# chinhau5/parallel_eda

Hardware: AMD Instinct MI355X
Metric: place+route wall-clock to feasibility (s/flow; bitcoin_miner-scale synthetic on stratixiv-like fabric) (lower is better)
Workload: dtype fp32; 1 GPU; model=bitcoin_miner, arch=bitcoin_stratixiv, grid=280x200, W=300, rr_nodes=15745036, rr_edges=87277236, blocks=37632, nets=35616, conns=110426, global_batch=110426, seq_len=0, final_overused=0, wirelength=4913966

## Files before the change

csrc/hip/place_kernel.hip:

```cpp
#include "pnr_hip.h"

namespace pnrh {

struct PlaceDev {
  const int32_t* net_blk_ptr;
  const int32_t* net_blks;
  const int32_t* blk_net_ptr;
  const int32_t* blk_nets;
  const int8_t* blk_type;
  const int8_t* tile_btype;
  const int32_t* type_cols;
  const int32_t* type_col_ptr;
  const uint8_t* fixed;
  const float* net_q;
  const int32_t* net_sink_ptr;
  const float* conn_crit;
  const float* delay_mat;
  int32_t* bx;
  int32_t* by;
  int32_t* bslot;
  int32_t* grid;
  float* net_cost;
  float* net_tcost;
  int32_t num_blocks, num_nets, gx, gy, cap, nx, ny, io_cap;
// ... 170 lines not shown
                     ? (p.tile_btype[tx * p.gy + ty] != p.blk_type[b])
                     : (is_io_loc(p, tx, ty) != (p.blk_type[b] == 0))) ok = 0;
        else if (cap_at(p, tx, ty) != 1) ok = 0;
        else {
          int32_t occ = p.grid[((int64_t)tx * p.gy + ty) * p.cap];
          if (occ >= 0 && p.macro_of[occ] != mid) ok = 0;
        }
      }
      if (ok) atomicAdd(&m.counters[0], 1);
    }
    ok = __shfl(ok, 0);
    if (!ok) return;
    float dbb = 0.0f, dtd = 0.0f;
    for (int32_t j = mm0; j < mm1; ++j) {
      int32_t b = p.macro_blk[j];
      for (int32_t k = p.blk_net_ptr[b] + lane; k < p.blk_net_ptr[b + 1];
           k += 64) {
        int32_t n = p.blk_nets[k];
        bool dup = false;
        for (int32_t j2 = mm0; j2 < j && !dup; ++j2)
          dup = blk_has_net(p, p.macro_blk[j2], n);
        if (dup) continue;
        dbb += net_bb_cost_macro(p, n, mid, ddx, ddy) - p.net_cost[n];
        if (timing_tradeoff > 0.0f)
          dtd += net_td_cost_macro(p, n, mid, ddx, ddy) - p.net_tcost[n];
      }
    }
    dbb = wave_sum_f32(dbb);
    dtd = wave_sum_f32(dtd);
    float delta = (1.0f - timing_tradeoff) * dbb * inv_bb_norm +
                  timing_tradeoff * dtd * inv_td_norm;
    bool accept;
    if (delta <= 0.0f) accept = true;
    else if (T <= 0.0f) accept = false;
    else {
      float u = (rng_hash(seed, batch, i * 131 + 5) & 0xFFFFFF) *
                (1.0f / 16777216.0f);
      accept = u < __expf(-delta / T);
    }
    if (!accept) return;
    if (lane == 0) {
      atomicAdd(&m.counters[1], 1);
      m.mv_blk[i] = blk;
      m.mv_to[i] = ((ddx + 4096) << 13) | (ddy + 4096);
      m.mv_other[i] = -2 - mid;
      m.mv_dbb[i] = dbb;
      m.mv_dtd[i] = dtd;
      m.mv_flags[i] = 1;
    }
    for (int32_t j = mm0; j < mm1; ++j) {
      int32_t b = p.macro_blk[j];
      for (int32_t k = p.blk_net_ptr[b] + lane; k < p.blk_net_ptr[b + 1];
           k += 64)
        atomicMin(&m.net_claim[p.blk_nets[k]], i);
    }
    for (int32_t j = mm0 + lane; j < mm1; j += 64) {
      int32_t b = p.macro_blk[j];
      atomicMin(&m.loc_claim[p.bx[b] * p.gy + p.by[b]], i);
      atomicMin(&m.loc_claim[(p.bx[b] + ddx) * p.gy + p.by[b] + ddy], i);
    }
    return;
  }
  int32_t other = p.grid[((int64_t)x1 * p.gy + y1) * p.cap + slot1];
  if (other == blk) return;
  if (other >= 0 && p.fixed && p.fixed[other]) return;
  if (other >= 0 && p.macro_of && p.macro_of[other] >= 0)
    return;
  if (lane == 0) atomicAdd(&m.counters[0], 1);
  float dbb = 0.0f, dtd = 0.0f;
  const int ox = other >= 0 ? x0 : -1000, oy = other >= 0 ? y0 : -1000;
  for (int32_t k = p.blk_net_ptr[blk] + lane; k < p.blk_net_ptr[blk + 1];
       k += 64) {
    int32_t n = p.blk_nets[k];
    dbb += net_bb_cost(p, n, blk, x1, y1, other, ox, oy) - p.net_cost[n];
    if (timing_tradeoff > 0.0f)
      dtd += net_td_cost(p, n, blk, x1, y1, other, ox, oy) - p.net_tcost[n];
  }
  if (other >= 0) {
    for (int32_t k = p.blk_net_ptr[other] + lane;
         k < p.blk_net_ptr[other + 1]; k += 64) {
      int32_t n = p.blk_nets[k];
      if (blk_has_net(p, blk, n)) continue;
      dbb += net_bb_cost(p, n, blk, x1, y1, other, ox, oy) - p.net_cost[n];
      if (timing_tradeoff > 0.0f)
        dtd += net_td_cost(p, n, blk, x1, y1, other, ox, oy) - p.net_tcost[n];
    }
  }
  dbb = wave_sum_f32(dbb);
  dtd = wave_sum_f32(dtd);
  float delta = (1.0f - timing_tradeoff) * dbb * inv_bb_norm +
                timing_tradeoff * dtd * inv_td_norm;
  bool accept;
  if (delta <= 0.0f) accept = true;
  else if (T <= 0.0f) accept = false;
  else {
    float u = (rng_hash(seed, batch, i * 131 + 5) & 0xFFFFFF) *
              (1.0f / 16777216.0f);
    accept = u < __expf(-delta / T);
  }
  if (!accept) return;
  if (lane == 0) {
    atomicAdd(&m.counters[1], 1);
    m.mv_blk[i] = blk;
    m.mv_to[i] = ((x1 * p.gy + y1) * p.cap + slot1);
    m.mv_other[i] = other;
    m.mv_dbb[i] = dbb;
    m.mv_dtd[i] = dtd;
    m.mv_flags[i] = 1;
    atomicMin(&m.loc_claim[x0 * p.gy + y0], i);
    atomicMin(&m.loc_claim[x1 * p.gy + y1], i);
  }
  for (int32_t k = p.blk_net_ptr[blk] + lane; k < p.blk_net_ptr[blk + 1];
       k += 64)
    atomicMin(&m.net_claim[p.blk_nets[k]], i);
  if (other >= 0)
    for (int32_t k = p.blk_net_ptr[other] + lane;
         k < p.blk_net_ptr[other + 1]; k += 64)
      atomicMin(&m.net_claim[p.blk_nets[k]], i);
}

__device__ int propose_select_impl(const PlaceDev& p, int rlim,
                                   uint32_t seed, uint32_t batch, int i,
                                   int& x1o, int& y1o, int& slot1o) {
  uint32_t r0 = rng_hash(seed ^ 0x5BD1E995u, batch, i);
  int32_t blk = r0 % p.num_blocks;
  if (p.fixed && p.fixed[blk]) return -1;
  if (p.rx0 >= 0 && (p.bx[blk] < p.rx0 || p.bx[blk] > p.rx1))
    return -1;
  bool io = p.blk_type[blk] == 0;
  int x0 = p.bx[blk], y0 = p.by[blk];
  int x1 = -1, y1 = -1, slot1 = 0;
  int bt = p.blk_type[blk];
  if (p.tile_btype && bt >= 2 && p.type_cols) {
    int c0 = p.type_col_ptr[bt - 2], c1 = p.type_col_ptr[bt - 1];
    int lo = c0, hi = c1;
    while (lo < hi) { int m = (lo + hi) >> 1;
                      if (p.type_cols[m] < x0 - rlim) lo = m + 1; else hi = m; }
    int lo2 = lo, hi2 = c1;
    while (lo2 < hi2) { int m = (lo2 + hi2) >> 1;
                        if (p.type_cols[m] <= x0 + rlim) lo2 = m + 1; else hi2 = m; }
    int ncol = lo2 - lo;
    if (ncol > 0) {
      int ylo = max(1, y0 - rlim), yhi = min(p.ny, y0 + rlim);
      for (int att = 0; att < 8; ++att) {
        uint32_t r1 = rng_hash(seed, batch, i * 131 + 7 * att + 1);
        uint32_t r2 = rng_hash(seed, batch, i * 131 + 7 * att + 2);
        int tx = p.type_cols[lo + (int)(r1 % ncol)];
        if (p.rx0 >= 0 && (tx < p.rx0 || tx > p.rx1)) continue;
        int ty = ylo + (int)(r2 % (yhi - ylo + 1));
        if (tx == x0 && ty == y0) continue;
        x1 = tx; y1 = ty; slot1 = 0;
        break;
      }
    }
  } else {
    for (int att = 0; att < 8; ++att) {
      uint32_t r1 = rng_hash(seed, batch, i * 131 + 7 * att + 1);
      uint32_t r2 = rng_hash(seed, batch, i * 131 + 7 * att + 2);
      int tx = x0 + (int)(r1 % (2 * rlim + 1)) - rlim;
      int ty = y0 + (int)(r2 % (2 * rlim + 1)) - rlim;
      if (tx < 0 || tx >= p.gx || ty < 0 || ty >= p.gy) continue;
      if (p.rx0 >= 0 && (tx < p.rx0 || tx > p.rx1)) continue;
      if (p.tile_btype) {
        if (p.tile_btype[tx * p.gy + ty] != p.blk_type[blk]) continue;
      } else if (is_io_loc(p, tx, ty) != io) continue;
      int c = cap_at(p, tx, ty);
      if (c <= 0) continue;
      if (tx == x0 && ty == y0) continue;
      x1 = tx; y1 = ty;
      slot1 = (int)(rng_hash(seed, batch, i * 131 + 7 * att + 3) % c);
      break;
    }
  }
  if (x1 < 0) return -1;
  x1o = x1; y1o = y1; slot1o = slot1;
  return blk;
}

__launch_bounds__(64 * PROP_WAVES, 2)
__global__ void place_resolve_kernel(PlaceDev p, MovesDev m) {
  const int lane = threadIdx.x & 63;
  const int i = blockIdx.x * PROP_WAVES + (threadIdx.x >> 6);
  if (i >= m.n_moves || m.mv_flags[i] != 1) return;
  int32_t blk = m.mv_blk[i];
  int32_t other = m.mv_other[i];
  int32_t to = m.mv_to[i];
  bool bad = false;
  if (other <= -2) {
    const int mid = -2 - other;
    const int ddx = (to >> 13) - 4096, ddy = (to & 0x1FFF) - 4096;
    const int32_t mm0 = p.macro_ptr[mid], mm1 = p.macro_ptr[mid + 1];
    for (int32_t j = mm0 + lane; j < mm1; j += 64) {
      int32_t b = p.macro_blk[j];
      int sx = p.bx[b], sy = p.by[b];
      if (m.loc_claim[sx * p.gy + sy] != i ||
          m.loc_claim[(sx + ddx) * p.gy + sy + ddy] != i) bad = true;
    }
    for (int32_t j = mm0; j < mm1; ++j) {
      int32_t b = p.macro_blk[j];
      for (int32_t k = p.blk_net_ptr[b] + lane; k < p.blk_net_ptr[b + 1];
           k += 64)
        if (m.net_claim[p.blk_nets[k]] != i) bad = true;
    }
  } else {
    int x1 = to / p.cap / p.gy, y1 = (to / p.cap) % p.gy;
    int x0 = p.bx[blk], y0 = p.by[blk];
    if (lane == 0 && (m.loc_claim[x0 * p.gy + y0] != i ||
                      m.loc_claim[x1 * p.gy + y1] != i)) bad = true;
    for (int32_t k = p.blk_net_ptr[blk] + lane; k < p.blk_net_ptr[blk + 1];
         k += 64)
      if (m.net_claim[p.blk_nets[k]] != i) bad = true;
    if (other >= 0)
      for (int32_t k = p.blk_net_ptr[other] + lane;
           k < p.blk_net_ptr[other + 1]; k += 64)
        if (m.net_claim[p.blk_nets[k]] != i) bad = true;
  }
  const bool win = !__any(bad);
  if (lane == 0) {
    if (!win) { m.mv_flags[i] = 0; atomicAdd(&m.counters[3], 1); }
    else { m.mv_flags[i] = 2; atomicAdd(&m.counters[2], 1); }
  }
}

__launch_bounds__(64 * PROP_WAVES, 2)
__global__ void place_apply_kernel(PlaceDev p, MovesDev m, float timing_tradeoff,
                                   double* cost_acc ) {
  const int lane = threadIdx.x & 63;
  const int i = blockIdx.x * PROP_WAVES + (threadIdx.x >> 6);
  if (i >= m.n_moves || m.mv_flags[i] != 2) return;
  int32_t blk = m.mv_blk[i];
  int32_t other = m.mv_other[i];
  int32_t to = m.mv_to[i];
  if (other <= -2) {
    const int mid = -2 - other;
    const int ddx = (to >> 13) - 4096, ddy = (to & 0x1FFF) - 4096;
    const int32_t mm0 = p.macro_ptr[mid], mm1 = p.macro_ptr[mid + 1];
    for (int32_t j = mm0; j < mm1; ++j) {
      int32_t b = p.macro_blk[j];
      for (int32_t k = p.blk_net_ptr[b] + lane; k < p.blk_net_ptr[b + 1];
           k += 64) {
        int32_t n = p.blk_nets[k];
        p.net_cost[n] = net_bb_cost_macro(p, n, mid, ddx, ddy);
        if (timing_tradeoff > 0.0f)
          p.net_tcost[n] = net_td_cost_macro(p, n, mid, ddx, ddy);
      }
    }
    if (lane == 0) {
      for (int32_t j = mm0; j < mm1; ++j) {
        int32_t b = p.macro_blk[j];
        p.grid[((int64_t)p.bx[b] * p.gy + p.by[b]) * p.cap + p.bslot[b]] = -1;
      }
      for (int32_t j = mm0; j < mm1; ++j) {
        int32_t b = p.macro_blk[j];
        int tx = p.bx[b] + ddx, ty = p.by[b] + ddy;
        p.grid[((int64_t)tx * p.gy + ty) * p.cap] = b;
        p.bx[b] = tx; p.by[b] = ty; p.bslot[b] = 0;
      }
      unsafeAtomicAdd(&cost_acc[0], (double)m.mv_dbb[i]);
      unsafeAtomicAdd(&cost_acc[1], (double)m.mv_dtd[i]);
    }
    return;
  }
  int slot1 = to % p.cap;
  int x1 = to / p.cap / p.gy, y1 = (to / p.cap) % p.gy;
  int x0 = p.bx[blk], y0 = p.by[blk], s0 = p.bslot[blk];
  const int ox = other >= 0 ? x0 : -1000, oy = other >= 0 ? y0 : -1000;
  for (int32_t k = p.blk_net_ptr[blk] + lane; k < p.blk_net_ptr[blk + 1];
       k += 64) {
    int32_t n = p.blk_nets[k];
    p.net_cost[n] = net_bb_cost(p, n, blk, x1, y1, other, ox, oy);
    if (timing_tradeoff > 0.0f)
      p.net_tcost[n] = net_td_cost(p, n, blk, x1, y1, other, ox, oy);
  }
  if (other >= 0)
    for (int32_t k = p.blk_net_ptr[other] + lane;
         k < p.blk_net_ptr[other + 1]; k += 64) {
      int32_t n = p.blk_nets[k];
      p.net_cost[n] = net_bb_cost(p, n, blk, x1, y1, other, ox, oy);
      if (timing_tradeoff > 0.0f)
        p.net_tcost[n] = net_td_cost(p, n, blk, x1, y1, other, ox, oy);
    }
  if (lane == 0) {
    p.grid[((int64_t)x0 * p.gy + y0) * p.cap + s0] = other >= 0 ? other : -1;
    p.grid[((int64_t)x1 * p.gy + y1) * p.cap + slot1] = blk;
    p.bx[blk] = x1; p.by[blk] = y1; p.bslot[blk] = slot1;
    if (other >= 0) { p.bx[other] = x0; p.by[other] = y0; p.bslot[other] = s0; }
    unsafeAtomicAdd(&cost_acc[0], (double)m.mv_dbb[i]);
    unsafeAtomicAdd(&cost_acc[1], (double)m.mv_dtd[i]);
  }
}

__global__ void place_reset_claims_kernel(int32_t* net_claim, int32_t nn,
                                          int32_t* loc_claim, int32_t nl,
                                          int32_t* counters) {
  int i = blockIdx.x * blockDim.x + threadIdx.x;
  int total = max(nn, nl);
  (void)counters;
  for (; i < total; i += gridDim.x * blockDim.x) {
    if (i < nn) net_claim[i] = 0x7FFFFFFF;
    if (i < nl) loc_claim[i] = 0x7FFFFFFF;
  }
}

__global__ void place_refresh_costs_kernel(PlaceDev p, float timing_tradeoff,
                                           double* out ) {
  int n = blockIdx.x * blockDim.x + threadIdx.x;
  for (; n < p.num_nets; n += gridDim.x * blockDim.x) {
    float c = net_bb_cost(p, n, -1, 0, 0, -1, 0, 0);
    p.net_cost[n] = c;
    unsafeAtomicAdd(&out[0], (double)c);
    float t = (timing_tradeoff > 0.0f)
                  ? net_td_cost(p, n, -1, 0, 0, -1, 0, 0) : 0.0f;
    p.net_tcost[n] = t;
    unsafeAtomicAdd(&out[1], (double)t);
  }
}

}

using namespace pnrh;

extern "C" {

struct PlaceLaunchArgs {
  const int32_t* net_blk_ptr; const int32_t* net_blks;
  const int32_t* blk_net_ptr; const int32_t* blk_nets;
  const int8_t* blk_type; const int8_t* tile_btype;
  const int32_t* type_cols; const int32_t* type_col_ptr;
  const uint8_t* fixed;
  const float* net_q;
  const int32_t* net_sink_ptr; const float* conn_crit; const float* delay_mat;
  int32_t* bx; int32_t* by; int32_t* bslot; int32_t* grid;
  float* net_cost; float* net_tcost;
  int32_t num_blocks, num_nets, gx, gy, cap, nx, ny, io_cap;
  int32_t rx0, rx1;
  const int32_t* macro_of; const int32_t* macro_ptr;
  const int32_t* macro_blk;
  int32_t* mv_blk; int32_t* mv_to; int32_t* mv_other;
  float* mv_dbb; float* mv_dtd; uint8_t* mv_flags;
  int32_t* net_claim; int32_t* loc_claim; int32_t* counters;
  int32_t n_moves;
  float T; int32_t rlim; float timing_tradeoff;
  float inv_bb_norm, inv_td_norm;
  uint32_t seed, batch;
  double* cost_acc;
};

static void unpack(const PlaceLaunchArgs* a, PlaceDev& p, MovesDev& m) {
  p.net_blk_ptr = a->net_blk_ptr; p.net_blks = a->net_blks;
  p.blk_net_ptr = a->blk_net_ptr; p.blk_nets = a->blk_nets;
  p.blk_type = a->blk_type; p.tile_btype = a->tile_btype;
  p.type_cols = a->type_cols; p.type_col_ptr = a->type_col_ptr;
  p.fixed = a->fixed;
  p.net_q = a->net_q;
  p.net_sink_ptr = a->net_sink_ptr; p.conn_crit = a->conn_crit;
  p.delay_mat = a->delay_mat;
  p.bx = a->bx; p.by = a->by; p.bslot = a->bslot; p.grid = a->grid;
  p.net_cost = a->net_cost; p.net_tcost = a->net_tcost;
  p.num_blocks = a->num_blocks; p.num_nets = a->num_nets;
  p.gx = a->gx; p.gy = a->gy; p.cap = a->cap;
  p.nx = a->nx; p.ny = a->ny; p.io_cap = a->io_cap;
  p.rx0 = a->rx0; p.rx1 = a->rx1;
  p.macro_of = a->macro_of; p.macro_ptr = a->macro_ptr;
  p.macro_blk = a->macro_blk;
  m.mv_blk = a->mv_blk; m.mv_to = a->mv_to; m.mv_other = a->mv_other;
  m.mv_dbb = a->mv_dbb; m.mv_dtd = a->mv_dtd; m.mv_flags = a->mv_flags;
  m.net_claim = a->net_claim; m.loc_claim = a->loc_claim;
  m.counters = a->counters; m.n_moves = a->n_moves;
}

int pnr_place_batch(const PlaceLaunchArgs* a, void* stream) {
  PlaceDev p; MovesDev m;
  unpack(a, p, m);
  hipStream_t s = (hipStream_t)stream;
  int rg = (max(max(a->num_nets, a->gx * a->gy), a->n_moves) + 255) / 256;
  rg = rg < 2048 ? rg : 2048;
  hipLaunchKernelGGL(place_reset_claims_kernel, dim3(rg), dim3(256), 0, s,
                     m.net_claim, p.num_nets, m.loc_claim, p.gx * p.gy,
                     m.counters);
  int mg = (m.n_moves + PROP_WAVES - 1) / PROP_WAVES;
  hipLaunchKernelGGL(place_propose_kernel, dim3(mg), dim3(64 * PROP_WAVES),
                     0, s, p, m, a->T, a->rlim, a->timing_tradeoff,
                     a->inv_bb_norm, a->inv_td_norm, a->seed, a->batch);
  hipLaunchKernelGGL(place_resolve_kernel, dim3(mg), dim3(64 * PROP_WAVES),
                     0, s, p, m);
  hipLaunchKernelGGL(place_apply_kernel, dim3(mg), dim3(64 * PROP_WAVES),
                     0, s, p, m, a->timing_tradeoff, a->cost_acc);
  return (int)hipGetLastError();
}

int pnr_place_refresh(const PlaceLaunchArgs* a, void* stream) {
  PlaceDev p; MovesDev m;
  unpack(a, p, m);
  hipStream_t s = (hipStream_t)stream;
  hipLaunchKernelGGL(place_refresh_costs_kernel, dim3(1024), dim3(256), 0, s,
                     p, a->timing_tradeoff, a->cost_acc);
  return (int)hipGetLastError();
}

int64_t pnr_place_args_sizeof() { return (int64_t)sizeof(PlaceLaunchArgs); }

}
```

parallel_eda_amd/place/gpu_placer.py:

```python
import ctypes as ct

import numpy as np

from ..arch.archdef import ArchDef
from ..ops import hip_api
from .placer import Placement, analytic_delay_matrix


class PlaceLaunchArgs(ct.Structure):
    _fields_ = [
        ("net_blk_ptr", ct.c_void_p), ("net_blks", ct.c_void_p),
        ("blk_net_ptr", ct.c_void_p), ("blk_nets", ct.c_void_p),
        ("blk_type", ct.c_void_p), ("tile_btype", ct.c_void_p),
        ("type_cols", ct.c_void_p), ("type_col_ptr", ct.c_void_p),
        ("fixed", ct.c_void_p),
        ("net_q", ct.c_void_p),
        ("net_sink_ptr", ct.c_void_p), ("conn_crit", ct.c_void_p),
        ("delay_mat", ct.c_void_p),
        ("bx", ct.c_void_p), ("by", ct.c_void_p), ("bslot", ct.c_void_p),
        ("grid", ct.c_void_p),
        ("net_cost", ct.c_void_p), ("net_tcost", ct.c_void_p),
        ("num_blocks", ct.c_int32), ("num_nets", ct.c_int32),
        ("gx", ct.c_int32), ("gy", ct.c_int32), ("cap", ct.c_int32),
        ("nx", ct.c_int32), ("ny", ct.c_int32), ("io_cap", ct.c_int32),
        ("rx0", ct.c_int32), ("rx1", ct.c_int32),
        ("macro_of", ct.c_void_p), ("macro_ptr", ct.c_void_p),
        ("macro_blk", ct.c_void_p),
        ("mv_blk", ct.c_void_p), ("mv_to", ct.c_void_p), ("mv_other", ct.c_void_p),
        ("mv_dbb", ct.c_void_p), ("mv_dtd", ct.c_void_p), ("mv_flags", ct.c_void_p),
        ("net_claim", ct.c_void_p), ("loc_claim", ct.c_void_p),
        ("counters", ct.c_void_p), ("n_moves", ct.c_int32),
        ("T", ct.c_float), ("rlim", ct.c_int32), ("timing_tradeoff", ct.c_float),
        ("inv_bb_norm", ct.c_float), ("inv_td_norm", ct.c_float),
        ("seed", ct.c_uint32), ("batch", ct.c_uint32),
        ("cost_acc", ct.c_void_p),
    ]


def _lib():
    lib = hip_api.lib()
    if not hasattr(lib, "_place_ready"):
        lib.pnr_place_batch.restype = ct.c_int
        lib.pnr_place_batch.argtypes = [ct.POINTER(PlaceLaunchArgs), ct.c_void_p]
        lib.pnr_place_refresh.restype = ct.c_int
        lib.pnr_place_refresh.argtypes = [ct.POINTER(PlaceLaunchArgs), ct.c_void_p]
        lib.pnr_place_args_sizeof.restype = ct.c_int64
        if lib.pnr_place_args_sizeof() != ct.sizeof(PlaceLaunchArgs):
            raise RuntimeError("PlaceLaunchArgs ABI mismatch")
        lib._place_ready = True
    return lib


def ptr(t):
    return ct.c_void_p(t.data_ptr())


class GpuPlacer:
    def __init__(self, netlist, arch: ArchDef, seed=7, timing=False,
                 device="cuda:0", n_moves=None, fixed=None,
                 delay_matrix="analytic", macros=None):
        import torch
        self.torch = torch
        self.device = device
        self.arch = arch
        self.nl = netlist
        self.seed = seed
        self.timing = timing
        nb = netlist.num_blocks
        nn = netlist.num_nets
        gx, gy = arch.nx + 2, arch.ny + 2
        self.gx, self.gy = gx, gy
        self.cap = max(1, arch.io_cap)
        self.batch_counter = 0

        counts = 1 + np.diff(netlist.net_sink_ptr)
        net_blk_ptr = np.r_[0, np.cumsum(counts)].astype(np.int32)
        net_blks = np.empty(net_blk_ptr[-1], dtype=np.int32)
        net_blks[net_blk_ptr[:-1]] = netlist.net_driver
        sidx = np.concatenate([
            np.arange(net_blk_ptr[i] + 1, net_blk_ptr[i + 1])
            for i in range(nn)]) if nn else np.zeros(0, dtype=np.int64)
        net_blks[sidx] = netlist.net_sinks
        net_of_member = np.repeat(np.arange(nn, dtype=np.int64),
                                  np.diff(net_blk_ptr))
        key = net_blks.astype(np.int64) * nn + net_of_member
        key = np.unique(key)
        mb = (key // nn).astype(np.int32)
        blk_nets = (key % nn).astype(np.int32)
        blk_net_ptr = np.zeros(nb + 1, dtype=np.int32)
        np.add.at(blk_net_ptr, mb + 1, 1)
        blk_net_ptr = np.cumsum(blk_net_ptr, dtype=np.int64).astype(np.int32)
        q = np.array([_cross_count(int(c)) for c in counts], dtype=np.float32)

        def up(a, dtype=None):
            t = torch.from_numpy(np.ascontiguousarray(a))
            return t.to(device)

        self.t_net_blk_ptr = up(net_blk_ptr)
        self.t_net_blks = up(net_blks)
        self.t_blk_net_ptr = up(blk_net_ptr)
        self.t_blk_nets = up(blk_nets)
        self.t_blk_type = up(netlist.block_type)
        self.t_tile_btype = (up(arch.tile_btype_grid())
                             if arch.is_heterogeneous() else None)
        self.t_type_cols = self.t_type_col_ptr = None
        if arch.is_heterogeneous():
            ram_cols = [x for x in range(1, arch.nx + 1)
                        if arch.col_block_type(x) == 2]
            dsp_cols = [x for x in range(1, arch.nx + 1)
                        if arch.col_block_type(x) == 3]
            self.t_type_cols = up(np.asarray(ram_cols + dsp_cols,
                                             dtype=np.int32))
            self.t_type_col_ptr = up(np.asarray(
                [0, len(ram_cols), len(ram_cols) + len(dsp_cols)],
                dtype=np.int32))
        self.t_net_q = up(q)
        self._fixed = fixed
        self.t_fixed = None
        if fixed is not None:
            mask = np.zeros(nb, dtype=np.uint8)
            mask[np.asarray(fixed[0], dtype=np.int64)] = 1
            self.t_fixed = up(mask)
        self.t_net_sink_ptr = up(netlist.net_sink_ptr.astype(np.int32))
        self.t_conn_crit = torch.zeros(netlist.num_conns, dtype=torch.float32,
                                       device=device)
        if timing:
            if delay_matrix == "routed":
                from .delay_matrix import routed_delay_matrix
                dm = routed_delay_matrix(arch)
            else:
                dm = analytic_delay_matrix(arch)
            self._dm = dm
            self.t_delay_mat = up(dm.ravel())
        else:
            self._dm = None
            self.t_delay_mat = None

        bx, by, bslot, grid = self._initial_placement(seed)
        self.t_macro_of = self.t_macro_ptr = self.t_macro_blk = None
        self.macros = macros or []
        if self.macros:
            bx, by, bslot, grid = self._legalize_macros(
                bx, by, bslot, grid, self.macros)
            macro_of = np.full(nb, -1, dtype=np.int32)
            mptr = [0]
            mblk = []
            for mi, grp in enumerate(self.macros):
                for (b, dx, dy) in grp:
                    macro_of[b] = mi
                    mblk.append(b)
                mptr.append(len(mblk))
            self.t_macro_of = up(macro_of)
            self.t_macro_ptr = up(np.asarray(mptr, dtype=np.int32))
            self.t_macro_blk = up(np.asarray(mblk, dtype=np.int32))
        self.t_bx = up(bx); self.t_by = up(by); self.t_bslot = up(bslot)
        self.t_grid = up(grid)
        self.t_net_cost = torch.zeros(nn, dtype=torch.float32, device=device)
        self.t_net_tcost = torch.zeros(nn, dtype=torch.float32, device=device)

        self.n_moves = n_moves or int(np.clip(nb // 16, 64, 1 << 16))
        nm = self.n_moves
        self.t_mv_blk = torch.zeros(nm, dtype=torch.int32, device=device)
        self.t_mv_to = torch.zeros(nm, dtype=torch.int32, device=device)
        self.t_mv_other = torch.zeros(nm, dtype=torch.int32, device=device)
        self.t_mv_dbb = torch.zeros(nm, dtype=torch.float32, device=device)
        self.t_mv_dtd = torch.zeros(nm, dtype=torch.float32, device=device)
        self.t_mv_flags = torch.zeros(nm, dtype=torch.uint8, device=device)
        self.t_net_claim = torch.zeros(nn, dtype=torch.int32, device=device)
        self.t_loc_claim = torch.zeros(gx * gy, dtype=torch.int32, device=device)
        self.t_counters = torch.zeros(4, dtype=torch.int32, device=device)
        self.t_cost_acc = torch.zeros(2, dtype=torch.float64, device=device)

        self.lib = _lib()
        self.bb_cost, self.td_cost = self.refresh_costs()

    def _initial_placement(self, seed):
        arch = self.arch
        nl = self.nl
        rng = np.random.default_rng(seed)
        nb = nl.num_blocks
        bx = np.zeros(nb, dtype=np.int32)
        by = np.zeros(nb, dtype=np.int32)
        bslot = np.zeros(nb, dtype=np.int32)
        if self._fixed is not None:
            bx2, by2, bs2, grid = self._initial_placement_free(rng)
            ids, fx, fy, fs = [np.asarray(a) for a in self._fixed]
            for b, x, y, sl in zip(ids, fx, fy, fs):
                occ = grid[x, y, sl]
                if occ == b:
                    continue
                grid[bx2[b], by2[b], bs2[b]] = occ
                if occ >= 0:
                    bx2[occ], by2[occ], bs2[occ] = bx2[b], by2[b], bs2[b]
                bx2[b], by2[b], bs2[b] = x, y, sl
                grid[x, y, sl] = b
            return bx2, by2, bs2, grid.reshape(-1)
        return self._initial_placement_free(rng, flat=True)

    def _legalize_macros(self, bx, by, bslot, grid, macros):
        arch = self.arch
        g = grid.reshape(self.gx, self.gy, self.cap)
        members = [b for grp in macros for (b, _, _) in grp]
        for b in members:
            g[bx[b], by[b], bslot[b]] = -1
        tb = (arch.tile_btype_grid().reshape(self.gx, self.gy)
              if arch.is_heterogeneous() else None)

        def tile_ok(b, x, y):
            if not (0 <= x < self.gx and 0 <= y < self.gy):
                return False
            bt = int(self.nl.block_type[b])
            if tb is not None:
                if tb[x, y] != bt:
                    return False
            else:
                io = (x == 0 or x == self.gx - 1 or
                      y == 0 or y == self.gy - 1)
                inner = 1 <= x <= arch.nx and 1 <= y <= arch.ny
                if bt == 0 or io or not inner:
                    return False
            return g[x, y, 0] < 0

        for grp in macros:
            placed = False
            for ax in range(1, arch.nx + 1):
                for ay in range(1, arch.ny + 1):
                    if all(tile_ok(b, ax + dx, ay + dy)
                           for (b, dx, dy) in grp):
                        for (b, dx, dy) in grp:
                            bx[b], by[b], bslot[b] = ax + dx, ay + dy, 0
                            g[ax + dx, ay + dy, 0] = b
                        placed = True
                        break
                if placed:
                    break
            if not placed:
                raise ValueError("cannot legalize macro (grid too full)")
        return bx, by, bslot, g.reshape(-1)

    def _initial_placement_free(self, rng, flat=False):
        arch = self.arch
        nl = self.nl
        nb = nl.num_blocks
        bx = np.zeros(nb, dtype=np.int32)
        by = np.zeros(nb, dtype=np.int32)
        bslot = np.zeros(nb, dtype=np.int32)
        grid = np.full((self.gx, self.gy, self.cap), -1, dtype=np.int32)
        ios = np.nonzero(nl.block_type == 0)[0]
        if not arch.is_heterogeneous():
            clbs = np.nonzero(nl.block_type == 1)[0]
            tiles = rng.permutation(arch.nx * arch.ny)[:len(clbs)]
            if len(tiles) < len(clbs):
                raise ValueError("too many CLBs for grid")
            bx[clbs] = tiles // arch.ny + 1
            by[clbs] = tiles % arch.ny + 1
            grid[bx[clbs], by[clbs], 0] = clbs
        else:
            col_t = np.asarray([arch.col_block_type(x)
                                for x in range(1, arch.nx + 1)])
            for t in (1, 2, 3):
                blks = np.nonzero(nl.block_type == t)[0]
                if not len(blks):
                    continue
                cols = np.nonzero(col_t == t)[0]
                cand = (cols[:, None] * arch.ny +
                        np.arange(arch.ny)[None, :]).ravel()
                if len(blks) > len(cand):
                    raise ValueError(f"too many type-{t} blocks for grid")
                tiles = cand[rng.permutation(len(cand))[:len(blks)]]
                bx[blks] = tiles // arch.ny + 1
                by[blks] = tiles % arch.ny + 1
                grid[bx[blks], by[blks], 0] = blks
        io_locs = ([(0, y) for y in range(1, arch.ny + 1)] +
                   [(self.gx - 1, y) for y in range(1, arch.ny + 1)] +
                   [(x, 0) for x in range(1, arch.nx + 1)] +
                   [(x, self.gy - 1) for x in range(1, arch.nx + 1)])
        slots = [(x, y, s) for (x, y) in io_locs for s in range(arch.io_cap)]
        sel = rng.permutation(len(slots))[:len(ios)]
        for b, k in zip(ios, sel):
            x, y, s = slots[k]
            bx[b], by[b], bslot[b] = x, y, s
            grid[x, y, s] = b
        return (bx, by, bslot, grid.reshape(-1)) if flat \
            else (bx, by, bslot, grid)

    def _args(self, T=0.0, rlim=1, tt=0.0, inv_bb=1.0, inv_td=1.0):
        a = PlaceLaunchArgs()
        a.net_blk_ptr = ptr(self.t_net_blk_ptr); a.net_blks = ptr(self.t_net_blks)
        a.blk_net_ptr = ptr(self.t_blk_net_ptr); a.blk_nets = ptr(self.t_blk_nets)
        a.blk_type = ptr(self.t_blk_type)
        a.tile_btype = (ptr(self.t_tile_btype)
                        if self.t_tile_btype is not None else None)
        a.type_cols = (ptr(self.t_type_cols)
                       if self.t_type_cols is not None else None)
        a.type_col_ptr = (ptr(self.t_type_col_ptr)
                          if self.t_type_col_ptr is not None else None)
        a.fixed = ptr(self.t_fixed) if self.t_fixed is not None else None
        a.net_q = ptr(self.t_net_q)
        a.net_sink_ptr = ptr(self.t_net_sink_ptr)
        a.conn_crit = ptr(self.t_conn_crit)
        a.delay_mat = ptr(self.t_delay_mat) if self.t_delay_mat is not None else None
        a.bx = ptr(self.t_bx); a.by = ptr(self.t_by); a.bslot = ptr(self.t_bslot)
        a.grid = ptr(self.t_grid)
        a.net_cost = ptr(self.t_net_cost); a.net_tcost = ptr(self.t_net_tcost)
        a.num_blocks = self.nl.num_blocks; a.num_nets = self.nl.num_nets
        a.gx = self.gx; a.gy = self.gy; a.cap = self.cap
        a.nx = self.arch.nx; a.ny = self.arch.ny; a.io_cap = self.arch.io_cap
        a.rx0, a.rx1 = getattr(self, "move_region", (-1, -1))
        if getattr(self, "t_macro_of", None) is not None:
            a.macro_of = ptr(self.t_macro_of)
            a.macro_ptr = ptr(self.t_macro_ptr)
            a.macro_blk = ptr(self.t_macro_blk)
        else:
            a.macro_of = a.macro_ptr = a.macro_blk = None
        a.mv_blk = ptr(self.t_mv_blk); a.mv_to = ptr(self.t_mv_to)
        a.mv_other = ptr(self.t_mv_other); a.mv_dbb = ptr(self.t_mv_dbb)
        a.mv_dtd = ptr(self.t_mv_dtd); a.mv_flags = ptr(self.t_mv_flags)
        a.net_claim = ptr(self.t_net_claim); a.loc_claim = ptr(self.t_loc_claim)
        a.counters = ptr(self.t_counters); a.n_moves = self.n_moves
        a.T = T; a.rlim = max(1, int(rlim)); a.timing_tradeoff = tt
        a.inv_bb_norm = inv_bb; a.inv_td_norm = inv_td
        a.seed = self.seed & 0xFFFFFFFF; a.batch = self.batch_counter
        a.cost_acc = ptr(self.t_cost_acc)
        return a

    def _stream(self):
        return self.torch.cuda.current_stream().cuda_stream

    def refresh_costs(self):
        self.t_cost_acc.zero_()
        a = self._args(tt=1.0 if self.timing else 0.0)
        rc = self.lib.pnr_place_refresh(ct.byref(a), self._stream())
        hip_api.check(rc, "place_refresh")
        self.torch.cuda.synchronize(self.device)
        bb, td = self.t_cost_acc.cpu().numpy()
        self.bb_cost, self.td_cost = float(bb), float(td)
        return self.bb_cost, self.td_cost

    def run_batches(self, T, rlim, target_moves, tt, bb_norm, td_norm,
                    max_batches=256):
        self.t_counters.zero_()
        batches = 0
        win = att = acc = 0
        while batches < max_batches:
            for _ in range(4):
                self.batch_counter += 1
                a = self._args(T=T, rlim=rlim, tt=tt,
                               inv_bb=1.0 / bb_norm, inv_td=1.0 / td_norm)
                rc = self.lib.pnr_place_batch(ct.byref(a), self._stream())
                hip_api.check(rc, "place_batch")
                batches += 1
            self.torch.cuda.synchronize(self.device)
            c = self.t_counters.cpu().numpy()
            att, acc, win = int(c[0]), int(c[1]), int(c[2])
            if win + (att - acc) >= target_moves:
                break
        else:
            self.torch.cuda.synchronize(self.device)
        srate = acc / max(1, att)
        return srate, att

    def set_move_region(self, x0, x1):
        self.move_region = (x0, x1)

    def set_crit(self, conn_crit):
        t = self.torch.from_numpy(np.ascontiguousarray(conn_crit,
                                                       dtype=np.float32))
        self.t_conn_crit.copy_(t.to(self.device))

    def placement(self):
        return Placement(self.t_bx.cpu().numpy(), self.t_by.cpu().numpy(),
                         self.t_bslot.cpu().numpy(),
                         bb_cost=self.bb_cost, td_cost=self.td_cost)

    def check_place(self):
        bx = self.t_bx.cpu().numpy(); by = self.t_by.cpu().numpy()
        bslot = self.t_bslot.cpu().numpy()
        grid = self.t_grid.cpu().numpy().reshape(self.gx, self.gy, self.cap)
        nl = self.nl
        tb = (self.arch.tile_btype_grid().reshape(self.gx, self.gy)
              if self.arch.is_heterogeneous() else None)
        for b in range(nl.num_blocks):
            x, y = bx[b], by[b]
            if tb is not None:
                if tb[x, y] != nl.block_type[b]:
                    return False, f"block {b} type/loc mismatch"
            else:
                io = nl.block_type[b] == 0
                on_io = (x == 0 or x == self.gx - 1 or y == 0 or
                         y == self.gy - 1)
                if io != on_io:
                    return False, f"block {b} type/loc mismatch"
            if grid[x, y, bslot[b]] != b:
                return False, f"grid inconsistent at block {b}"
        occ = (grid >= 0).sum()
        if occ != nl.num_blocks:
            return False, f"grid count {occ} != blocks {nl.num_blocks}"
        for grp in getattr(self, "macros", []):
            b0, dx0, dy0 = grp[0]
            for (b, dx, dy) in grp[1:]:
                if (bx[b] - bx[b0] != dx - dx0 or
                        by[b] - by[b0] != dy - dy0):
                    return False, f"macro offsets broken at block {b}"
        return True, ""


def _cross_count(n):
    q3, q50 = 1.0, 2.79
    if n <= 3:
        return q3
    if n >= 50:
        return q50 + 0.02616 * (n - 50)
    return q3 + (q50 - q3) * (n - 3) / 47.0


def anneal_place_gpu(netlist, arch, seed=7, timing_tradeoff=0.5, inner_num=1.0,
                     sta=None, crit_exp=1.0, verbose=False, device="cuda:0",
                     n_moves=None, fixed=None, delay_matrix="analytic",
                     macros=None):
    timing = sta is not None and timing_tradeoff > 0
    placer = GpuPlacer(netlist, arch, seed=seed, timing=timing, device=device,
                       n_moves=n_moves, fixed=fixed, delay_matrix=delay_matrix,
                       macros=macros)
    nb = netlist.num_blocks
    move_lim = max(256, int(inner_num * (nb ** 1.3333)))
    rlim = float(max(arch.nx, arch.ny))
    tt = timing_tradeoff if timing else 0.0

    def refresh_crit():
        if not timing:
            return
        bx = placer.t_bx.cpu().numpy(); by = placer.t_by.cpu().numpy()
        drv = netlist.net_driver
        d_per_conn = np.empty(netlist.num_conns, dtype=np.float32)
        dm = placer._dm if placer._dm is not None else analytic_delay_matrix(arch)
        net_of_conn = np.repeat(np.arange(netlist.num_nets),
                                np.diff(netlist.net_sink_ptr))
        dx = np.abs(bx[netlist.net_sinks] - bx[drv[net_of_conn]])
        dy = np.abs(by[netlist.net_sinks] - by[drv[net_of_conn]])
        d_per_conn = dm[dx, dy]
        cpd, slack, c = sta.analyze(d_per_conn)
        placer.set_crit(np.asarray(c) ** crit_exp)
        placer.refresh_costs()

    refresh_crit()
    norm_mode = tt > 0

    def norms():
        if norm_mode:
            return (max(placer.bb_cost, 1e-12), max(placer.td_cost, 1e-30))
        return (1.0, 1.0)

    bb_norm, td_norm = norms()
    placer.run_batches(1e30, rlim, min(move_lim, 2048), tt, bb_norm, td_norm,
                       max_batches=16)
    torch = placer.torch
    flags = placer.t_mv_flags
    sel = flags >= 1
    if int(sel.sum().item()) >= 8:
        d = (1.0 - tt) * placer.t_mv_dbb[sel] / bb_norm
        if tt > 0:
            d = d + tt * placer.t_mv_dtd[sel] / td_norm
        t = float(20.0 * d.std().item())
    else:
        t = 20.0 * placer.bb_cost / max(1, netlist.num_nets) / bb_norm
    placer.refresh_costs()
    if t <= 0:
        t = 1.0
    history = []
    itemp = 0
    while True:
        refresh_crit()
        bb_norm, td_norm = norms()
        srate, _ = placer.run_batches(t, rlim, move_lim, tt, bb_norm, td_norm)
        placer.refresh_costs()
        cost = placer.bb_cost
        history.append((t, cost, srate, rlim))
        if verbose:
            print(f"[gpu] T={t:.3e} bb={cost:.1f} acc={srate:.2f} rlim={rlim:.0f}")
        if srate > 0.96:
            t *= 0.5
        elif srate > 0.8:
            t *= 0.9
        elif srate > 0.15 or rlim > 1:
            t *= 0.95
        else:
            t *= 0.8
        rlim = min(max(rlim * (1.0 - 0.44 + srate), 1.0),
                   float(max(arch.nx, arch.ny)))
        itemp += 1
        exit_cost = 1.0 if norm_mode else cost
        if t < 0.005 * exit_cost / max(1, netlist.num_nets):
            break
        if itemp > 500:
            break
    placer.run_batches(0.0, 1.0, move_lim, tt, bb_norm, td_norm)
    placer.refresh_costs()
    ok, err = placer.check_place()
    if not ok:
        raise RuntimeError(f"gpu check_place failed: {err}")
    pl = placer.placement()
    pl.stats = {"temps": itemp, "move_lim": move_lim, "history": history,
                "engine": "gpu"}
    return pl
```

Measured before the change: 8.115 s.

## Run placement batches on-device with epoch-keyed 64-bit claims and in-kernel termination

```diff
diff --git a/csrc/hip/place_kernel.hip b/csrc/hip/place_kernel.hip
--- a/csrc/hip/place_kernel.hip
+++ b/csrc/hip/place_kernel.hip
@@ -496,6 +496,314 @@
   }
 }
 
+struct RunDev {
+  int32_t* mv_from;
+  unsigned long long* net_claim;
+  unsigned long long* loc_claim;
+  int32_t* ctrl;
+};
+
+__device__ __forceinline__ unsigned long long claim_key(uint32_t batch, int i) {
+  return ((unsigned long long)batch << 32) | (0xFFFFFFFFu - (uint32_t)i);
+}
+
+__launch_bounds__(64 * PROP_WAVES, 2)
+__global__ void place_propose_run_kernel(PlaceDev p, MovesDev m, RunDev r,
+                                         float T, int rlim,
+                                         float timing_tradeoff,
+                                         float inv_bb_norm, float inv_td_norm,
+                                         uint32_t seed, uint32_t batch) {
+  if (r.ctrl[0]) return;
+  const int lane = threadIdx.x & 63;
+  const int i = blockIdx.x * PROP_WAVES + (threadIdx.x >> 6);
+  if (i >= m.n_moves) return;
+  const unsigned long long key = claim_key(batch, i);
+  int sel = -1, sx1 = -1, sy1 = -1, sslot = 0;
+  if (lane == 0) {
+    m.mv_flags[i] = 0;
+    sel = propose_select_impl(p, rlim, seed, batch, i, sx1, sy1, sslot);
+  }
+  sel = __shfl(sel, 0);
+  if (sel < 0) return;
+  const int x1 = __shfl(sx1, 0);
+  const int y1 = __shfl(sy1, 0);
+  const int slot1 = __shfl(sslot, 0);
+  const int32_t blk = sel;
+  const int x0 = p.bx[blk], y0 = p.by[blk];
+  const int mid = p.macro_of ? p.macro_of[blk] : -1;
+  if (mid >= 0) {
+    const int ddx = x1 - x0, ddy = y1 - y0;
+    const int32_t mm0 = p.macro_ptr[mid], mm1 = p.macro_ptr[mid + 1];
+    if (mm1 - mm0 > 16) return;
+    int ok = 0;
+    if (lane == 0) {
+      ok = 1;
+      for (int32_t j = mm0; j < mm1 && ok; ++j) {
+        int32_t b = p.macro_blk[j];
+        int sx = p.bx[b], sy = p.by[b];
+        int tx = sx + ddx, ty = sy + ddy;
+        if (p.fixed && p.fixed[b]) ok = 0;
+        else if (tx < 0 || tx >= p.gx || ty < 0 || ty >= p.gy) ok = 0;
+        else if (p.rx0 >= 0 && (tx < p.rx0 || tx > p.rx1 ||
+                                sx < p.rx0 || sx > p.rx1)) ok = 0;
+        else if (p.tile_btype
+                     ? (p.tile_btype[tx * p.gy + ty] != p.blk_type[b])
+                     : (is_io_loc(p, tx, ty) != (p.blk_type[b] == 0))) ok = 0;
+        else if (cap_at(p, tx, ty) != 1) ok = 0;
+        else {
+          int32_t occ = p.grid[((int64_t)tx * p.gy + ty) * p.cap];
+          if (occ >= 0 && p.macro_of[occ] != mid) ok = 0;
+        }
+      }
+      if (ok) atomicAdd(&m.counters[0], 1);
+    }
+    ok = __shfl(ok, 0);
+    if (!ok) return;
+    float dbb = 0.0f, dtd = 0.0f;
+    for (int32_t j = mm0; j < mm1; ++j) {
+      int32_t b = p.macro_blk[j];
+      for (int32_t k = p.blk_net_ptr[b] + lane; k < p.blk_net_ptr[b + 1];
+           k += 64) {
+        int32_t n = p.blk_nets[k];
+        bool dup = false;
+        for (int32_t j2 = mm0; j2 < j && !dup; ++j2)
+          dup = blk_has_net(p, p.macro_blk[j2], n);
+        if (dup) continue;
+        dbb += net_bb_cost_macro(p, n, mid, ddx, ddy) - p.net_cost[n];
+        if (timing_tradeoff > 0.0f)
+          dtd += net_td_cost_macro(p, n, mid, ddx, ddy) - p.net_tcost[n];
+      }
+    }
+    dbb = wave_sum_f32(dbb);
+    dtd = wave_sum_f32(dtd);
+    float delta = (1.0f - timing_tradeoff) * dbb * inv_bb_norm +
+                  timing_tradeoff * dtd * inv_td_norm;
+    bool accept;
+    if (delta <= 0.0f) accept = true;
+    else if (T <= 0.0f) accept = false;
+    else {
+      float u = (rng_hash(seed, batch, i * 131 + 5) & 0xFFFFFF) *
+                (1.0f / 16777216.0f);
+      accept = u < __expf(-delta / T);
+    }
+    if (!accept) return;
+    if (lane == 0) {
+      atomicAdd(&m.counters[1], 1);
+      m.mv_blk[i] = blk;
+      m.mv_to[i] = ((ddx + 4096) << 13) | (ddy + 4096);
+      m.mv_other[i] = -2 - mid;
+      m.mv_dbb[i] = dbb;
+      m.mv_dtd[i] = dtd;
+      m.mv_flags[i] = 1;
+      r.mv_from[i] = x0 * p.gy + y0;
+    }
+    for (int32_t j = mm0; j < mm1; ++j) {
+      int32_t b = p.macro_blk[j];
+      for (int32_t k = p.blk_net_ptr[b] + lane; k < p.blk_net_ptr[b + 1];
+           k += 64)
+        atomicMax(&r.net_claim[p.blk_nets[k]], key);
+    }
+    for (int32_t j = mm0 + lane; j < mm1; j += 64) {
+      int32_t b = p.macro_blk[j];
+      atomicMax(&r.loc_claim[p.bx[b] * p.gy + p.by[b]], key);
+      atomicMax(&r.loc_claim[(p.bx[b] + ddx) * p.gy + p.by[b] + ddy], key);
+    }
+    return;
+  }
+  int32_t other = p.grid[((int64_t)x1 * p.gy + y1) * p.cap + slot1];
+  if (other == blk) return;
+  if (other >= 0 && p.fixed && p.fixed[other]) return;
+  if (other >= 0 && p.macro_of && p.macro_of[other] >= 0)
+    return;
+  if (lane == 0) atomicAdd(&m.counters[0], 1);
+  float dbb = 0.0f, dtd = 0.0f;
+  const int ox = other >= 0 ? x0 : -1000, oy = other >= 0 ? y0 : -1000;
+  for (int32_t k = p.blk_net_ptr[blk] + lane; k < p.blk_net_ptr[blk + 1];
+       k += 64) {
+    int32_t n = p.blk_nets[k];
+    dbb += net_bb_cost(p, n, blk, x1, y1, other, ox, oy) - p.net_cost[n];
+    if (timing_tradeoff > 0.0f)
+      dtd += net_td_cost(p, n, blk, x1, y1, other, ox, oy) - p.net_tcost[n];
+  }
+  if (other >= 0) {
+    for (int32_t k = p.blk_net_ptr[other] + lane;
+         k < p.blk_net_ptr[other + 1]; k += 64) {
+      int32_t n = p.blk_nets[k];
+      if (blk_has_net(p, blk, n)) continue;
+      dbb += net_bb_cost(p, n, blk, x1, y1, other, ox, oy) - p.net_cost[n];
+      if (timing_tradeoff > 0.0f)
+        dtd += net_td_cost(p, n, blk, x1, y1, other, ox, oy) - p.net_tcost[n];
+    }
+  }
+  dbb = wave_sum_f32(dbb);
+  dtd = wave_sum_f32(dtd);
+  float delta = (1.0f - timing_tradeoff) * dbb * inv_bb_norm +
+                timing_tradeoff * dtd * inv_td_norm;
+  bool accept;
+  if (delta <= 0.0f) accept = true;
+  else if (T <= 0.0f) accept = false;
+  else {
+    float u = (rng_hash(seed, batch, i * 131 + 5) & 0xFFFFFF) *
+              (1.0f / 16777216.0f);
+    accept = u < __expf(-delta / T);
+  }
+  if (!accept) return;
+  if (lane == 0) {
+    atomicAdd(&m.counters[1], 1);
+    m.mv_blk[i] = blk;
+    m.mv_to[i] = ((x1 * p.gy + y1) * p.cap + slot1);
+    m.mv_other[i] = other;
+    m.mv_dbb[i] = dbb;
+    m.mv_dtd[i] = dtd;
+    m.mv_flags[i] = 1;
+    r.mv_from[i] = x0 * p.gy + y0;
+    atomicMax(&r.loc_claim[x0 * p.gy + y0], key);
+    atomicMax(&r.loc_claim[x1 * p.gy + y1], key);
+  }
+  for (int32_t k = p.blk_net_ptr[blk] + lane; k < p.blk_net_ptr[blk + 1];
+       k += 64)
+    atomicMax(&r.net_claim[p.blk_nets[k]], key);
+  if (other >= 0)
+    for (int32_t k = p.blk_net_ptr[other] + lane;
+         k < p.blk_net_ptr[other + 1]; k += 64)
+      atomicMax(&r.net_claim[p.blk_nets[k]], key);
+}
+
+__device__ void commit_move(const PlaceDev& p, const MovesDev& m,
+                            const RunDev& r, float timing_tradeoff,
+                            double* cost_acc, uint32_t batch) {
+  const int lane = threadIdx.x & 63;
+  const int i = blockIdx.x * PROP_WAVES + (threadIdx.x >> 6);
+  if (i >= m.n_moves || m.mv_flags[i] != 1) return;
+  const unsigned long long key = claim_key(batch, i);
+  int32_t blk = m.mv_blk[i];
+  int32_t other = m.mv_other[i];
+  int32_t to = m.mv_to[i];
+  bool bad = false;
+  if (other <= -2) {
+    const int mid = -2 - other;
+    const int ddx = (to >> 13) - 4096, ddy = (to & 0x1FFF) - 4096;
+    const int32_t mm0 = p.macro_ptr[mid], mm1 = p.macro_ptr[mid + 1];
+    for (int32_t j = mm0 + lane; j < mm1; j += 64) {
+      int32_t b = p.macro_blk[j];
+      int sx = p.bx[b], sy = p.by[b];
+      int tx = sx + ddx, ty = sy + ddy;
+      if (tx < 0 || tx >= p.gx || ty < 0 || ty >= p.gy) bad = true;
+      else if (r.loc_claim[sx * p.gy + sy] != key ||
+               r.loc_claim[tx * p.gy + ty] != key) bad = true;
+    }
+    for (int32_t j = mm0; j < mm1; ++j) {
+      int32_t b = p.macro_blk[j];
+      for (int32_t k = p.blk_net_ptr[b] + lane; k < p.blk_net_ptr[b + 1];
+           k += 64)
+        if (r.net_claim[p.blk_nets[k]] != key) bad = true;
+    }
+  } else {
+    int x1 = to / p.cap / p.gy, y1 = (to / p.cap) % p.gy;
+    if (lane == 0 && (r.loc_claim[r.mv_from[i]] != key ||
+                      r.loc_claim[x1 * p.gy + y1] != key)) bad = true;
+    for (int32_t k = p.blk_net_ptr[blk] + lane; k < p.blk_net_ptr[blk + 1];
+         k += 64)
+      if (r.net_claim[p.blk_nets[k]] != key) bad = true;
+    if (other >= 0)
+      for (int32_t k = p.blk_net_ptr[other] + lane;
+           k < p.blk_net_ptr[other + 1]; k += 64)
+        if (r.net_claim[p.blk_nets[k]] != key) bad = true;
+  }
+  const bool win = !__any(bad);
+  if (lane == 0) {
+    if (!win) { m.mv_flags[i] = 0; atomicAdd(&m.counters[3], 1); }
+    else { m.mv_flags[i] = 2; atomicAdd(&m.counters[2], 1); }
+  }
+  if (!win) return;
+  if (other <= -2) {
+    const int mid = -2 - other;
+    const int ddx = (to >> 13) - 4096, ddy = (to & 0x1FFF) - 4096;
+    const int32_t mm0 = p.macro_ptr[mid], mm1 = p.macro_ptr[mid + 1];
+    for (int32_t j = mm0; j < mm1; ++j) {
+      int32_t b = p.macro_blk[j];
+      for (int32_t k = p.blk_net_ptr[b] + lane; k < p.blk_net_ptr[b + 1];
+           k += 64) {
+        int32_t n = p.blk_nets[k];
+        p.net_cost[n] = net_bb_cost_macro(p, n, mid, ddx, ddy);
+        if (timing_tradeoff > 0.0f)
+          p.net_tcost[n] = net_td_cost_macro(p, n, mid, ddx, ddy);
+      }
+    }
+    if (lane == 0) {
+      for (int32_t j = mm0; j < mm1; ++j) {
+        int32_t b = p.macro_blk[j];
+        p.grid[((int64_t)p.bx[b] * p.gy + p.by[b]) * p.cap + p.bslot[b]] = -1;
+      }
+      for (int32_t j = mm0; j < mm1; ++j) {
+        int32_t b = p.macro_blk[j];
+        int tx = p.bx[b] + ddx, ty = p.by[b] + ddy;
+        p.grid[((int64_t)tx * p.gy + ty) * p.cap] = b;
+        p.bx[b] = tx; p.by[b] = ty; p.bslot[b] = 0;
+      }
+      unsafeAtomicAdd(&cost_acc[0], (double)m.mv_dbb[i]);
+      unsafeAtomicAdd(&cost_acc[1], (double)m.mv_dtd[i]);
+    }
+    return;
+  }
+  int slot1 = to % p.cap;
+  int x1 = to / p.cap / p.gy, y1 = (to / p.cap) % p.gy;
+  int x0 = p.bx[blk], y0 = p.by[blk], s0 = p.bslot[blk];
+  const int ox = other >= 0 ? x0 : -1000, oy = other >= 0 ? y0 : -1000;
+  for (int32_t k = p.blk_net_ptr[blk] + lane; k < p.blk_net_ptr[blk + 1];
+       k += 64) {
+    int32_t n = p.blk_nets[k];
+    p.net_cost[n] = net_bb_cost(p, n, blk, x1, y1, other, ox, oy);
+    if (timing_tradeoff > 0.0f)
+      p.net_tcost[n] = net_td_cost(p, n, blk, x1, y1, other, ox, oy);
+  }
+  if (other >= 0)
+    for (int32_t k = p.blk_net_ptr[other] + lane;
+         k < p.blk_net_ptr[other + 1]; k += 64) {
+      int32_t n = p.blk_nets[k];
+      p.net_cost[n] = net_bb_cost(p, n, blk, x1, y1, other, ox, oy);
+      if (timing_tradeoff > 0.0f)
+        p.net_tcost[n] = net_td_cost(p, n, blk, x1, y1, other, ox, oy);
+    }
+  if (lane == 0) {
+    p.grid[((int64_t)x0 * p.gy + y0) * p.cap + s0] = other >= 0 ? other : -1;
+    p.grid[((int64_t)x1 * p.gy + y1) * p.cap + slot1] = blk;
+    p.bx[blk] = x1; p.by[blk] = y1; p.bslot[blk] = slot1;
+    if (other >= 0) { p.bx[other] = x0; p.by[other] = y0; p.bslot[other] = s0; }
+    unsafeAtomicAdd(&cost_acc[0], (double)m.mv_dbb[i]);
+    unsafeAtomicAdd(&cost_acc[1], (double)m.mv_dtd[i]);
+  }
+}
+
+__launch_bounds__(64 * PROP_WAVES, 2)
+__global__ void place_commit_kernel(PlaceDev p, MovesDev m, RunDev r,
+                                    float timing_tradeoff, double* cost_acc,
+                                    uint32_t batch, int check,
+                                    int32_t target_moves) {
+  if (r.ctrl[0]) return;
+  commit_move(p, m, r, timing_tradeoff, cost_acc, batch);
+  if (!check) return;
+  asm volatile("s_waitcnt vmcnt(0)" ::: "memory");
+  __syncthreads();
+  if (threadIdx.x != 0) return;
+  __threadfence();
+  asm volatile("s_waitcnt vmcnt(0)" ::: "memory");
+  int ticket = __hip_atomic_fetch_add(&r.ctrl[2], 1, __ATOMIC_RELAXED,
+                                      __HIP_MEMORY_SCOPE_AGENT);
+  if (ticket != (int)gridDim.x - 1) return;
+  __threadfence();
+  int att = __hip_atomic_load(&m.counters[0], __ATOMIC_RELAXED,
+                              __HIP_MEMORY_SCOPE_AGENT);
+  int acc = __hip_atomic_load(&m.counters[1], __ATOMIC_RELAXED,
+                              __HIP_MEMORY_SCOPE_AGENT);
+  int win = __hip_atomic_load(&m.counters[2], __ATOMIC_RELAXED,
+                              __HIP_MEMORY_SCOPE_AGENT);
+  r.ctrl[1] += 4;
+  if (win + (att - acc) >= target_moves) r.ctrl[0] = 1;
+  __hip_atomic_store(&r.ctrl[2], 0, __ATOMIC_RELAXED,
+                     __HIP_MEMORY_SCOPE_AGENT);
+}
+
 __global__ void place_refresh_costs_kernel(PlaceDev p, float timing_tradeoff,
                                            double* out ) {
   int n = blockIdx.x * blockDim.x + threadIdx.x;
@@ -538,6 +846,9 @@
   float inv_bb_norm, inv_td_norm;
   uint32_t seed, batch;
   double* cost_acc;
+  int32_t* mv_from;
+  unsigned long long* net_claim64; unsigned long long* loc_claim64;
+  int32_t* run_ctrl;
 };
 
 static void unpack(const PlaceLaunchArgs* a, PlaceDev& p, MovesDev& m) {
@@ -583,6 +894,32 @@
   return (int)hipGetLastError();
 }
 
+int pnr_place_run(const PlaceLaunchArgs* a, uint32_t first_batch,
+                  int32_t target_moves, int32_t n_batches, void* stream) {
+  if (n_batches < 0 || (n_batches & 3) || first_batch == 0 ||
+      !a->mv_from || !a->net_claim64 || !a->loc_claim64 || !a->run_ctrl)
+    return (int)hipErrorInvalidValue;
+  PlaceDev p; MovesDev m;
+  unpack(a, p, m);
+  RunDev r;
+  r.mv_from = a->mv_from;
+  r.net_claim = a->net_claim64; r.loc_claim = a->loc_claim64;
+  r.ctrl = a->run_ctrl;
+  hipStream_t s = (hipStream_t)stream;
+  int mg = (m.n_moves + PROP_WAVES - 1) / PROP_WAVES;
+  for (int32_t k = 0; k < n_batches; ++k) {
+    const uint32_t batch = first_batch + (uint32_t)k;
+    hipLaunchKernelGGL(place_propose_run_kernel, dim3(mg),
+                       dim3(64 * PROP_WAVES), 0, s, p, m, r, a->T, a->rlim,
+                       a->timing_tradeoff, a->inv_bb_norm, a->inv_td_norm,
+                       a->seed, batch);
+    hipLaunchKernelGGL(place_commit_kernel, dim3(mg), dim3(64 * PROP_WAVES),
+                       0, s, p, m, r, a->timing_tradeoff, a->cost_acc, batch,
+                       (int)(((k + 1) & 3) == 0), target_moves);
+  }
+  return (int)hipGetLastError();
+}
+
 int pnr_place_refresh(const PlaceLaunchArgs* a, void* stream) {
   PlaceDev p; MovesDev m;
   unpack(a, p, m);
diff --git a/parallel_eda_amd/place/gpu_placer.py b/parallel_eda_amd/place/gpu_placer.py
--- a/parallel_eda_amd/place/gpu_placer.py
+++ b/parallel_eda_amd/place/gpu_placer.py
@@ -1,4 +1,5 @@
 import ctypes as ct
+import math
 
 import numpy as np
 
@@ -34,7 +35,13 @@
         ("inv_bb_norm", ct.c_float), ("inv_td_norm", ct.c_float),
         ("seed", ct.c_uint32), ("batch", ct.c_uint32),
         ("cost_acc", ct.c_void_p),
+        ("mv_from", ct.c_void_p),
+        ("net_claim64", ct.c_void_p), ("loc_claim64", ct.c_void_p),
+        ("run_ctrl", ct.c_void_p),
     ]
+
+
+RUN_CHUNK_BATCHES = 32
 
 
 def _lib():
@@ -42,6 +49,9 @@
     if not hasattr(lib, "_place_ready"):
         lib.pnr_place_batch.restype = ct.c_int
         lib.pnr_place_batch.argtypes = [ct.POINTER(PlaceLaunchArgs), ct.c_void_p]
+        lib.pnr_place_run.restype = ct.c_int
+        lib.pnr_place_run.argtypes = [ct.POINTER(PlaceLaunchArgs), ct.c_uint32,
+                                      ct.c_int32, ct.c_int32, ct.c_void_p]
         lib.pnr_place_refresh.restype = ct.c_int
         lib.pnr_place_refresh.argtypes = [ct.POINTER(PlaceLaunchArgs), ct.c_void_p]
         lib.pnr_place_args_sizeof.restype = ct.c_int64
@@ -58,9 +68,10 @@
 class GpuPlacer:
     def __init__(self, netlist, arch: ArchDef, seed=7, timing=False,
                  device="cuda:0", n_moves=None, fixed=None,
-                 delay_matrix="analytic", macros=None):
+                 delay_matrix="analytic", macros=None, legacy_batches=False):
         import torch
         self.torch = torch
+        self.legacy_batches = legacy_batches
         self.device = device
         self.arch = arch
         self.nl = netlist
@@ -77,10 +88,9 @@
         net_blk_ptr = np.r_[0, np.cumsum(counts)].astype(np.int32)
         net_blks = np.empty(net_blk_ptr[-1], dtype=np.int32)
         net_blks[net_blk_ptr[:-1]] = netlist.net_driver
-        sidx = np.concatenate([
-            np.arange(net_blk_ptr[i] + 1, net_blk_ptr[i + 1])
-            for i in range(nn)]) if nn else np.zeros(0, dtype=np.int64)
-        net_blks[sidx] = netlist.net_sinks
+        is_sink = np.ones(len(net_blks), dtype=bool)
+        is_sink[net_blk_ptr[:-1]] = False
+        net_blks[is_sink] = netlist.net_sinks
         net_of_member = np.repeat(np.arange(nn, dtype=np.int64),
                                   np.diff(net_blk_ptr))
         key = net_blks.astype(np.int64) * nn + net_of_member
@@ -90,7 +100,7 @@
         blk_net_ptr = np.zeros(nb + 1, dtype=np.int32)
         np.add.at(blk_net_ptr, mb + 1, 1)
         blk_net_ptr = np.cumsum(blk_net_ptr, dtype=np.int64).astype(np.int32)
-        q = np.array([_cross_count(int(c)) for c in counts], dtype=np.float32)
+        q = _cross_count_vec(counts).astype(np.float32)
 
         def up(a, dtype=None):
             t = torch.from_numpy(np.ascontiguousarray(a))
@@ -166,9 +176,21 @@
         self.t_mv_dbb = torch.zeros(nm, dtype=torch.float32, device=device)
         self.t_mv_dtd = torch.zeros(nm, dtype=torch.float32, device=device)
         self.t_mv_flags = torch.zeros(nm, dtype=torch.uint8, device=device)
-        self.t_net_claim = torch.zeros(nn, dtype=torch.int32, device=device)
-        self.t_loc_claim = torch.zeros(gx * gy, dtype=torch.int32, device=device)
-        self.t_counters = torch.zeros(4, dtype=torch.int32, device=device)
+        self.t_net_claim = self.t_loc_claim = None
+        self.t_net_claim64 = self.t_loc_claim64 = None
+        if legacy_batches:
+            self.t_net_claim = torch.zeros(nn, dtype=torch.int32, device=device)
+            self.t_loc_claim = torch.zeros(gx * gy, dtype=torch.int32,
+                                           device=device)
+        else:
+            self.t_net_claim64 = torch.zeros(nn, dtype=torch.int64,
+                                             device=device)
+            self.t_loc_claim64 = torch.zeros(gx * gy, dtype=torch.int64,
+                                             device=device)
+        self.t_mv_from = torch.zeros(nm, dtype=torch.int32, device=device)
+        self.t_run_state = torch.zeros(8, dtype=torch.int32, device=device)
+        self.t_counters = self.t_run_state[:4]
+        self.t_run_ctrl = self.t_run_state[4:]
         self.t_cost_acc = torch.zeros(2, dtype=torch.float64, device=device)
 
         self.lib = _lib()
@@ -316,7 +338,16 @@
         a.mv_blk = ptr(self.t_mv_blk); a.mv_to = ptr(self.t_mv_to)
         a.mv_other = ptr(self.t_mv_other); a.mv_dbb = ptr(self.t_mv_dbb)
         a.mv_dtd = ptr(self.t_mv_dtd); a.mv_flags = ptr(self.t_mv_flags)
-        a.net_claim = ptr(self.t_net_claim); a.loc_claim = ptr(self.t_loc_claim)
+        if self.legacy_batches:
+            a.net_claim = ptr(self.t_net_claim)
+            a.loc_claim = ptr(self.t_loc_claim)
+            a.net_claim64 = a.loc_claim64 = None
+        else:
+            a.net_claim = a.loc_claim = None
+            a.net_claim64 = ptr(self.t_net_claim64)
+            a.loc_claim64 = ptr(self.t_loc_claim64)
+        a.mv_from = ptr(self.t_mv_from)
+        a.run_ctrl = ptr(self.t_run_ctrl)
         a.counters = ptr(self.t_counters); a.n_moves = self.n_moves
         a.T = T; a.rlim = max(1, int(rlim)); a.timing_tradeoff = tt
         a.inv_bb_norm = inv_bb; a.inv_td_norm = inv_td
@@ -339,6 +370,35 @@
 
     def run_batches(self, T, rlim, target_moves, tt, bb_norm, td_norm,
                     max_batches=256):
+        if self.legacy_batches:
+            return self._run_batches_legacy(T, rlim, target_moves, tt,
+                                            bb_norm, td_norm, max_batches)
+        self.t_run_state.zero_()
+        a = self._args(T=T, rlim=rlim, tt=tt,
+                       inv_bb=1.0 / bb_norm, inv_td=1.0 / td_norm)
+        target = int(min(max(math.ceil(target_moves), -0x7FFFFFFF),
+                         0x7FFFFFFF))
+        cap = 4 * ((max_batches + 3) // 4)
+        first = self.batch_counter + 1
+        enq = 0
+        att = acc = executed = 0
+        while enq < cap:
+            n = min(RUN_CHUNK_BATCHES, cap - enq)
+            rc = self.lib.pnr_place_run(ct.byref(a), first + enq, target, n,
+                                        self._stream())
+            hip_api.check(rc, "place_run")
+            enq += n
+            st = self.t_run_state.cpu().numpy()
+            att, acc = int(st[0]), int(st[1])
+            done, executed = int(st[4]), int(st[5])
+            if done:
+                break
+        self.batch_counter += executed
+        srate = acc / max(1, att)
+        return srate, att
+
+    def _run_batches_legacy(self, T, rlim, target_moves, tt, bb_norm, td_norm,
+                            max_batches=256):
         self.t_counters.zero_()
         batches = 0
         win = att = acc = 0
@@ -380,19 +440,20 @@
         nl = self.nl
         tb = (self.arch.tile_btype_grid().reshape(self.gx, self.gy)
               if self.arch.is_heterogeneous() else None)
-        for b in range(nl.num_blocks):
-            x, y = bx[b], by[b]
-            if tb is not None:
-                if tb[x, y] != nl.block_type[b]:
-                    return False, f"block {b} type/loc mismatch"
-            else:
-                io = nl.block_type[b] == 0
-                on_io = (x == 0 or x == self.gx - 1 or y == 0 or
-                         y == self.gy - 1)
-                if io != on_io:
-                    return False, f"block {b} type/loc mismatch"
-            if grid[x, y, bslot[b]] != b:
-                return False, f"grid inconsistent at block {b}"
+        btype = np.asarray(nl.block_type)
+        if tb is not None:
+            bad_type = tb[bx, by] != btype
+        else:
+            on_io = ((bx == 0) | (bx == self.gx - 1) | (by == 0) |
+                     (by == self.gy - 1))
+            bad_type = (btype == 0) != on_io
+        bad_grid = grid[bx, by, bslot] != np.arange(nl.num_blocks)
+        bad = bad_type | bad_grid
+        if bad.any():
+            b = int(np.argmax(bad))
+            if bad_type[b]:
+                return False, f"block {b} type/loc mismatch"
+            return False, f"grid inconsistent at block {b}"
         occ = (grid >= 0).sum()
         if occ != nl.num_blocks:
             return False, f"grid count {occ} != blocks {nl.num_blocks}"
@@ -414,14 +475,22 @@
     return q3 + (q50 - q3) * (n - 3) / 47.0
 
 
+def _cross_count_vec(counts):
+    n = np.asarray(counts, dtype=np.int64)
+    q3, q50 = 1.0, 2.79
+    return np.where(n <= 3, q3,
+                    np.where(n >= 50, q50 + 0.02616 * (n - 50),
+                             q3 + (q50 - q3) * (n - 3) / 47.0))
+
+
 def anneal_place_gpu(netlist, arch, seed=7, timing_tradeoff=0.5, inner_num=1.0,
                      sta=None, crit_exp=1.0, verbose=False, device="cuda:0",
                      n_moves=None, fixed=None, delay_matrix="analytic",
-                     macros=None):
+                     macros=None, legacy_batches=False):
     timing = sta is not None and timing_tradeoff > 0
     placer = GpuPlacer(netlist, arch, seed=seed, timing=timing, device=device,
                        n_moves=n_moves, fixed=fixed, delay_matrix=delay_matrix,
-                       macros=macros)
+                       macros=macros, legacy_batches=legacy_batches)
     nb = netlist.num_blocks
     move_lim = max(256, int(inner_num * (nb ** 1.3333)))
     rlim = float(max(arch.nx, arch.ny))
```

After: 7.710 s, median of 6. 5.0% less time.
